# hzxie/Stereo-3D-Reconstruction

Hardware: AMD Instinct MI355X
Metric: stereo pairs/s forward (batch 32, 224x224 -> 32^3 voxel) (higher is better)
Workload: dtype f32

## Files before the change

### stereo-3d-reconstruction_amd/csrc/s3r_conv_wino.hip

```cpp
#include "s3r_kernels.h"
#include <cstdlib>

namespace s3r {

typedef float wf32x16 __attribute__((ext_vector_type(16)));
typedef float wv2f __attribute__((ext_vector_type(2)));
template <int N> struct WVec;
template <> struct WVec<1> { typedef float type; };
template <> struct WVec<2> { typedef wv2f type; };
typedef float wv4f __attribute__((ext_vector_type(4)));
template <> struct WVec<4> { typedef wv4f type; };
template <int N>
__device__ __forceinline__ float wvget(const typename WVec<N>::type& v, int i) {
    if constexpr (N == 1) return v; else return v[i];
}

#define S3R_LDS_PTR_W(p) ((__attribute__((address_space(3))) void*)(p))

#ifndef S3R_WNB
#define S3R_WNB 2
#endif
#ifndef S3R_WBK
#define S3R_WBK 32
#endif
// ... 610 lines not shown
template <int VEC, int KIND, bool HEAD = false, bool XM = false>
__global__ __launch_bounds__(256, (KIND == 1 ? 4 : 3)) void wino_dual_kernel(const ConvParams p) {
    extern __shared__ __attribute__((aligned(16))) float wsmem[];
    if ((int)blockIdx.x < p.big_wgs)
        wino_body<VEC, KIND, 2, false, HEAD, XM>(p, blockIdx.x, p.big_wgs, p.n_begin, p.n_cut, wsmem);
    else
        wino_body<VEC, KIND, 2, true, false, XM>(p, (int)blockIdx.x - p.big_wgs, (int)gridDim.x - p.big_wgs, p.n_cut, p.n_end, wsmem);
}

template <int KIND, bool HEAD>
__global__ __launch_bounds__(256) void wino_finish_kernel(const ConvParams p, const int n_begin, const int n_end, const int npad) {
    constexpr bool DECONV = KIND == 2;
    constexpr int NCLS = WinoKind<KIND>::NCLS, R = WinoKind<KIND>::R;
    const int S = p.Nd * p.Nh * p.Nw;
    const int nn = n_end - n_begin;
    const int pc = DECONV ? (int)blockIdx.y : 0;
    const int rd = (pc >> 2) & 1, rh = (pc >> 1) & 1, rw = pc & 1;
    const float lo = p.act == ACT_RELU ? 0.f : -__builtin_inff();
    constexpr int NBLK = DECONV ? 8 * NCLS : NCLS;
    const int ntl = npad >> 6;
    const float* __restrict__ base = p.part + (size_t)pc * NCLS * 64;
    auto blk = [&](int mm, int nl) { return base + ((size_t)mm * ntl + (nl >> 6)) * (NBLK * 64) + (nl & 63); };
    const long long total = HEAD ? nn : (long long)p.Cout * nn;
    for (long long i = (long long)blockIdx.x * 256 + threadIdx.x; i < total; i += (long long)gridDim.x * 256) {
        const int mrow = HEAD ? 0 : (int)(i / nn);
        const int nl = (int)(i - (long long)mrow * nn);
        const int n = n_begin + nl;
        const int b = p.dS.div(n);
        int rem = n - b * S;
        const int pd = p.dHW.div(rem);
        rem -= pd * p.Nh * p.Nw;
        const int q = p.dW.div(rem);
        const int pw = rem - q * p.Nw;
        int e0, row1 = R;
        if constexpr (DECONV)
            e0 = b * p.y_bs + p.y_org + (2 * pd * p.y_ds + 2 * q * p.y_hs + pw) * 2 + rd * p.y_ds + rh * p.y_hs + rw;
        else {
            e0 = b * p.y_bs + p.y_org + pd * p.y_ds + R * q * p.y_hs + pw;
            row1 = p.Hout - R * q;
        }
        if constexpr (HEAD) {
            float tw[2][R];
#pragma unroll
            for (int wm = 0; wm < 2; ++wm) {
                float th[2][R];
#pragma unroll
                for (int hh = 0; hh < 2; ++hh) {
#pragma unroll
                    for (int k = 0; k < R; ++k) th[hh][k] = 0.f;
                    for (int r = 0; r < 16; ++r) {
                        const int mm = 32 * wm + 4 * hh + (r & 3) + 8 * (r >> 2);
                        if (mm >= p.Cout) continue;
                        const float sc = p.scale ? p.scale[mm] : 1.f, sf = p.shift ? p.shift[mm] : 0.f, hw = p.head_w[mm];
                        float m[NCLS], y[R];
#pragma unroll
                        for (int c = 0; c < NCLS; ++c) m[c] = blk(mm, nl)[c * 64];
                        wino_out<KIND>(m, y);
#pragma unroll
                        for (int k = 0; k < R; ++k) th[hh][k] = fmaf(wino_act(y[k], sc, sf, lo), hw, th[hh][k]);
                    }
                }
#pragma unroll
                for (int k = 0; k < R; ++k) tw[wm][k] = th[0][k] + th[1][k];
            }
            const float hsc = p.head_scale ? p.head_scale[0] : 1.f, hsf = p.head_shift ? p.head_shift[0] : 0.f;
#pragma unroll
            for (int k = 0; k < R; ++k)
                p.y[e0 + wino_out_off<KIND>(k, p.y_ds, p.y_hs)] = wino_head_act(fmaf(tw[0][k] + tw[1][k], hsc, hsf), p.head_act);
        } else {
            const float sc = p.scale ? p.scale[mrow] : 1.f, sf = p.shift ? p.shift[mrow] : 0.f;
            float m[NCLS], y[R];
#pragma unroll
            for (int c = 0; c < NCLS; ++c) m[c] = blk(mrow, nl)[c * 64];
            wino_out<KIND>(m, y);
            float* __restrict__ yo = p.y + (size_t)mrow * p.y_cs + e0;
#pragma unroll
            for (int k = 0; k < R; ++k)
                if (k < row1) yo[wino_out_off<KIND>(k, p.y_ds, p.y_hs)] = wino_act(y[k], sc, sf, lo);
        }
    }
}

template <int KIND>
static hipError_t launch_wino_finish(const ConvParams& p, int n_begin, int n_end, int npad, hipStream_t stream) {
    const long long total = p.head_w ? (long long)(n_end - n_begin) : (long long)p.Cout * (n_end - n_begin);
    const long long blocks = (total + 255) / 256;
    const dim3 grid((unsigned)(blocks < 8192 ? blocks : 8192), KIND == 2 ? 8 : 1);
    if constexpr (KIND == 2) {
        if (p.head_w) hipLaunchKernelGGL((wino_finish_kernel<KIND, true>), grid, dim3(256), 0, stream, p, n_begin, n_end, npad);
        else hipLaunchKernelGGL((wino_finish_kernel<KIND, false>), grid, dim3(256), 0, stream, p, n_begin, n_end, npad);
    } else {
        hipLaunchKernelGGL((wino_finish_kernel<KIND, false>), grid, dim3(256), 0, stream, p, n_begin, n_end, npad);
    }
    return hipGetLastError();
}

constexpr int WCN = 64;
#ifdef S3R_ABLATE
static int wabl_mode() { static const int m = getenv("S3R_ABL") ? atoi(getenv("S3R_ABL")) : 0; return m; }
#define S3R_WABL(p) (p).debug = wabl_mode()
#else
#define S3R_WABL(p) (void)0
#endif

int64_t wino_slab_elems(int kind, int cout, int ntotal, const WinoLaunch& L) {
    if (L.mode == WINO_SERIAL) return 0;
    const int ncls = kind == 2 ? 72 : 6;
    const int n0 = L.mode == WINO_DUAL ? L.n_cut : 0;
    const int64_t npad = (int64_t)((ntotal - n0 + WCN - 1) / WCN) * WCN;
    return (int64_t)ncls * cout * npad;
}

WinoLaunch wino_plan(int kind, int cout, int kcls, int ntotal, bool head, int forced) {
    WinoLaunch L;
    L.mode = WINO_SERIAL; L.n_cut = 0;
    const int m_tiles = (cout + WBM - 1) / WBM;
    const int pcs = kind == 2 ? 8 : 1;
    const int ncls = kind == 2 ? 9 : 6;
    const long W = (long)m_tiles * ((ntotal + WCN - 1) / WCN) * pcs;
    if (forced < 0) {
        static const int env_mode = getenv("S3R_WINO_FORM") ? atoi(getenv("S3R_WINO_FORM")) : -1;
        forced = env_mode;
    }
    const int occ = kind == 2 ? 3 : 4;
    const int CUS = cu_count();
    const double u = (double)W / (double)CUS;
    int kb = (int)u;
    if (forced >= 0) {
        L.mode = forced <= WINO_DUAL ? forced : WINO_SERIAL;
        if ((double)kb >= u) kb -= 1;
    } else {
        (void)head;
        constexpr double EFF = 0.9, EFF_ALONE = 0.7, SLAB = 100.0, LAUNCH = 220.0, TAIL = 0.6;
        const double unit = (double)ncls * kcls;
        auto serial_cost = [&](int w) {
            const int rem = w % occ;
            return (w - (rem == 1 ? 1 : 0)) * unit / EFF + (rem == 1 ? unit / EFF_ALONE : 0.0);
        };
        const double serial = serial_cost((int)__builtin_ceil(u));
        const double cp = __builtin_ceil(u * ncls) * (kcls / EFF + SLAB) + LAUNCH;
        double best = serial;
        if (cp < best) { best = cp; L.mode = WINO_CP; }
        for (int k : {(int)u, (int)u % occ == 1 ? (int)u - 1 : 0}) {
            if (k < 1 || (double)k >= u) continue;
            const double dual = serial_cost(k) + TAIL * __builtin_ceil((u - k) * ncls) * (kcls / EFF + SLAB) + LAUNCH;
            if (dual < 0.97 * best) { best = dual; L.mode = WINO_DUAL; kb = k; }
        }
    }
    if (L.mode == WINO_DUAL) {
        const long n_main = ((long)kb * CUS) / (m_tiles * pcs);
        L.n_cut = (int)(n_main * WCN);
        if (L.n_cut <= 0 || L.n_cut >= ntotal) { L.mode = L.n_cut <= 0 ? WINO_CP : WINO_SERIAL; L.n_cut = 0; }
    }
    return L;
}

template <int VEC, int KIND>
static hipError_t launch_wino_forms(ConvParams p, const WinoLaunch& L, hipStream_t stream) {
    const int ntotal = p.Ntotal;
    if (p.out_mode && (KIND != 2 || L.mode != WINO_CP)) return hipErrorInvalidValue;
    auto lds_of = [](int bn) { return (size_t)WNB * WBK * (WBM + (KIND == 2 ? 2 : 1) * bn) * sizeof(float); };
    const int pcs = KIND == 2 ? 8 : 1;
    constexpr int NCLS = WinoKind<KIND>::NCLS;
    p.n_begin = 0; p.n_end = ntotal;
    if (L.mode == WINO_SERIAL) {
        const dim3 grid(p.m_tiles * ((ntotal + WCN - 1) / WCN) * pcs);
        if constexpr (KIND == 2) {
            if (p.head_w) {
                if (p.xd_mode) hipLaunchKernelGGL((wino_kernel<VEC, KIND, 2, false, true, true>), grid, dim3(256), lds_of(WCN), stream, p);
                else hipLaunchKernelGGL((wino_kernel<VEC, KIND, 2, false, true, false>), grid, dim3(256), lds_of(WCN), stream, p);
            } else {
                if (p.xd_mode) hipLaunchKernelGGL((wino_kernel<VEC, KIND, 2, false, false, true>), grid, dim3(256), lds_of(WCN), stream, p);
                else hipLaunchKernelGGL((wino_kernel<VEC, KIND, 2, false, false, false>), grid, dim3(256), lds_of(WCN), stream, p);
            }
            return hipGetLastError();
        }
        hipLaunchKernelGGL((wino_kernel<VEC, KIND, 2, false, false>), grid, dim3(256), lds_of(WCN), stream, p);
        return hipGetLastError();
    }
    if (!p.part) return hipErrorInvalidValue;
    const int n0 = L.mode == WINO_DUAL ? L.n_cut : 0;
    const int cp_tiles = (ntotal - n0 + WCN - 1) / WCN;
    const int cp_wgs = p.m_tiles * cp_tiles * NCLS * pcs;
    if (L.mode == WINO_DUAL) {
        p.n_cut = n0;
        p.big_wgs = p.m_tiles * (n0 / WCN) * pcs;
        const dim3 grid(p.big_wgs + cp_wgs);
        if constexpr (KIND == 2) {
            if (p.head_w) {
                if (p.xd_mode) hipLaunchKernelGGL((wino_dual_kernel<VEC, KIND, true, true>), grid, dim3(256), lds_of(WCN), stream, p);
                else hipLaunchKernelGGL((wino_dual_kernel<VEC, KIND, true, false>), grid, dim3(256), lds_of(WCN), stream, p);
            } else {
                if (p.xd_mode) hipLaunchKernelGGL((wino_dual_kernel<VEC, KIND, false, true>), grid, dim3(256), lds_of(WCN), stream, p);
                else hipLaunchKernelGGL((wino_dual_kernel<VEC, KIND, false, false>), grid, dim3(256), lds_of(WCN), stream, p);
            }
        } else {
            hipLaunchKernelGGL((wino_dual_kernel<VEC, KIND>), grid, dim3(256), lds_of(WCN), stream, p);
        }
    } else if (KIND == 2 && p.xd_mode) {
        hipLaunchKernelGGL((wino_kernel<VEC, KIND, 2, true, false, KIND == 2>), dim3(cp_wgs), dim3(256), lds_of(WCN), stream, p);
    } else {
        hipLaunchKernelGGL((wino_kernel<VEC, KIND, 2, true, false>), dim3(cp_wgs), dim3(256), lds_of(WCN), stream, p);
    }
    hipError_t e = hipGetLastError();
    if (e != hipSuccess) return e;
    if (p.out_mode) return launch_wino_handoff(p, 2, p.out_mode - 1, cp_tiles * WCN, stream);
    AuxScope aux(stream, 4.0 * (double)(ntotal - n0) * p.Cout * (pcs * NCLS + (p.head_w ? 0.0 : pcs * WinoKind<KIND>::R)));
    return launch_wino_finish<KIND>(p, n0, ntotal, cp_tiles * WCN, stream);
}

hipError_t launch_conv_wino(ConvParams p, const WinoLaunch& L, hipStream_t stream, int* launches) {
    if (p.Cin % WBK != 0 || p.stride != 1 || p.transposed || p.ksplit != 1 || p.head_w || p.act == ACT_SIGMOID)
        return hipErrorInvalidValue;
    p.kh = 1;
    S3R_WABL(p);
    p.m_tiles = (p.Cout + WBM - 1) / WBM;
    if (launches) *launches = L.mode == WINO_SERIAL ? 1 : 2;
    return p.Nw % 4 == 0 ? launch_wino_forms<4, 1>(p, L, stream) : launch_wino_forms<1, 1>(p, L, stream);
}

hipError_t launch_deconv_wino(ConvParams p, const WinoLaunch& L, hipStream_t stream, int* launches) {
    if (p.Cin % WBK != 0 || !p.transposed || p.ksplit != 1 || !p.xd || p.act == ACT_SIGMOID || (p.head_w && p.Cout > WBM))
        return hipErrorInvalidValue;
    S3R_WABL(p);
    p.m_tiles = (p.Cout + WBM - 1) / WBM;
    if (launches) *launches = L.mode == WINO_SERIAL ? 1 : 2;
    if (p.Nw % 4 != 0) return hipErrorInvalidValue;
    return launch_wino_forms<4, 2>(p, L, stream);
}

template <int AX> struct WAxis;
template <> struct WAxis<0> { static constexpr int N = 6, M = 4, R = 3; };
template <> struct WAxis<1> { static constexpr int N = 5, M = 2, R = 4; };
int wino2_classes(int ax) { return ax == 1 ? 25 : 36; }
int wino2_outputs(int ax) { return ax == 1 ? 2 : 4; }

template <int AX>
__device__ __forceinline__ void wax_bt(const float (&r)[WAxis<AX>::N], float (&v)[WAxis<AX>::N]) {
    if constexpr (AX == 0) wino_rows_to_classes<4>(r, v);
    else {
        v[0] = fmaf(2.f, r[0] - r[2], r[3] - r[1]);
        v[1] = fmaf(-2.f, r[1], r[3] - r[2]);
        v[2] = fmaf(2.f, r[1], fmaf(-3.f, r[2], r[3]));
        v[3] = r[3] - r[1];
        v[4] = fmaf(2.f, r[1] - r[3], r[4] - r[2]);
    }
}
template <int AX>
__device__ __forceinline__ void wax_at(const float (&m)[WAxis<AX>::N], float (&y)[WAxis<AX>::M]) {
    if constexpr (AX == 0) wino_out<1>(m, y);
    else {
        y[0] = ((m[0] + m[1]) + m[2]) + m[3];
        y[1] = fmaf(2.f, m[3], m[1] - m[2]) + m[4];
    }
}
template <int AX>
__device__ __forceinline__ float wax_g(int c, const float (&g)[WAxis<AX>::R]) {
    if constexpr (AX == 0) {
        const float s02 = g[0] + g[2], a = g[0] * (1.f / 24.f) + g[2] * (1.f / 6.f), b12 = g[1] * (1.f / 12.f);
        return c == 0 ? g[0] * 0.25f : c == 1 ? (s02 + g[1]) * (-1.f / 6.f) : c == 2 ? (s02 - g[1]) * (-1.f / 6.f)
             : c == 3 ? a + b12 : c == 4 ? a - b12 : g[2];
    } else {
        const float e = g[0] + g[2], o = g[1] + g[3];
        return c == 0 ? g[0] * 0.5f : c == 1 ? (e + o) * -0.5f : c == 2 ? (o - e) * (1.f / 6.f)
             : c == 3 ? fmaf(g[3], 4.f / 3.f, fmaf(g[2], 2.f / 3.f, fmaf(g[1], 1.f / 3.f, g[0] * (1.f / 6.f)))) : g[3];
    }
}

template <int AX>
__global__ __launch_bounds__(256) void wino2_input_kernel(const float* __restrict__ x, float* __restrict__ V, unsigned total,
                                                          int Dp, int Hp, int Wp, int SD, int SH, FastDiv dW, FastDiv dSH, FastDiv dSD) {
    constexpr int N = WAxis<AX>::N, M = WAxis<AX>::M;
    for (unsigned i = blockIdx.x * 256u + threadIdx.x; i < total; i += gridDim.x * 256u) {
        const unsigned row = (unsigned)dW.div((int)i);
        const int w = (int)(i - row * (unsigned)Wp);
        const unsigned pg = (unsigned)dSH.div((int)row);
        const int sh = (int)(row - pg * (unsigned)SH);
        const unsigned pl = (unsigned)dSD.div((int)pg);
        const int sd = (int)(pg - pl * (unsigned)SD);
        const float* __restrict__ src = x + ((size_t)pl * Dp + M * sd) * Hp * Wp + (size_t)M * sh * Wp + w;
        float t[N][N];
#pragma unroll
        for (int a = 0; a < N; ++a) {
            float r[N], v[N];
#pragma unroll
            for (int b = 0; b < N; ++b)
                r[b] = (M * sd + a < Dp && M * sh + b < Hp) ? src[((size_t)a * Hp + b) * Wp] : 0.f;
            wax_bt<AX>(r, v);
#pragma unroll
            for (int b = 0; b < N; ++b) t[a][b] = v[b];
        }
#pragma unroll
        for (int b = 0; b < N; ++b) {
            float r[N], v[N];
#pragma unroll
            for (int a = 0; a < N; ++a) r[a] = t[a][b];
            wax_bt<AX>(r, v);
#pragma unroll
            for (int a = 0; a < N; ++a) V[(size_t)(a * N + b) * total + i] = v[a];
        }
    }
}

hipError_t launch_wino2_input(const float* x, float* V, int ax, long long planes, int Dp, int Hp, int Wp, int SD, int SH, hipStream_t s) {
    const long long total = planes * SD * SH * Wp;
    if (total >= (1ll << 31) || (ax != 0 && ax != 1)) return hipErrorInvalidValue;
    const long long blocks = (total + 255) / 256;
    const dim3 grid((unsigned)(blocks < 16384 ? blocks : 16384));
    const FastDiv dW((unsigned)Wp), dSH((unsigned)SH), dSD((unsigned)SD);
    if (ax == 0) hipLaunchKernelGGL(wino2_input_kernel<0>, grid, dim3(256), 0, s, x, V, (unsigned)total, Dp, Hp, Wp, SD, SH, dW, dSH, dSD);
    else hipLaunchKernelGGL(wino2_input_kernel<1>, grid, dim3(256), 0, s, x, V, (unsigned)total, Dp, Hp, Wp, SD, SH, dW, dSH, dSD);
    return hipGetLastError();
}

template <int AX>
__global__ void pack_wino2_kernel(const float* __restrict__ w, float* __restrict__ wp, int Cin, int Cout, int CoutPad) {
    constexpr int N = WAxis<AX>::N, R = WAxis<AX>::R;
    const size_t per_cls = (size_t)R * Cin * CoutPad;
    for (size_t i = blockIdx.x * (size_t)blockDim.x + threadIdx.x; i < (size_t)N * N * per_cls; i += (size_t)gridDim.x * blockDim.x) {
        const int cls = (int)(i / per_cls);
        const int ca = cls / N, cb = cls - ca * N;
        size_t r = i % per_cls;
        const int co = (int)(r % CoutPad);
        r /= CoutPad;
        const int c = (int)(r % WBK);
        r /= WBK;
        const int tw = (int)(r % R);
        const int cc = (int)(r / R);
        const int cin = cc * WBK + c;
        float v = 0.f;
        if (co < Cout) {
            const float* g = w + ((size_t)co * Cin + cin) * R * R * R + tw;
            float gd[R];
#pragma unroll
            for (int kd = 0; kd < R; ++kd) {
                float gh[R];
#pragma unroll
                for (int kh = 0; kh < R; ++kh) gh[kh] = g[(kd * R + kh) * R];
                gd[kd] = wax_g<AX>(cb, gh);
            }
            v = wax_g<AX>(ca, gd);
        }
        wp[i] = v;
    }
}

__global__ void pack_wino2p_kernel(const float* __restrict__ w, float* __restrict__ wp, int Cin, int Cout, int CoutPad);
hipError_t launch_pack_wino2(const float* w, float* wp, int ax, int Cin, int Cout, int CoutPad, hipStream_t s) {
    if (ax == 0) hipLaunchKernelGGL(pack_wino2_kernel<0>, dim3(1024), dim3(256), 0, s, w, wp, Cin, Cout, CoutPad);
    else if (ax == 1) hipLaunchKernelGGL(pack_wino2_kernel<1>, dim3(1024), dim3(256), 0, s, w, wp, Cin, Cout, CoutPad);
    else if (ax == 2) hipLaunchKernelGGL(pack_wino2p_kernel, dim3(1024), dim3(256), 0, s, w, wp, Cin, Cout, CoutPad);
    else return hipErrorInvalidValue;
    return hipGetLastError();
}

__device__ __forceinline__ void wino2_copy_out(const float* __restrict__ lds, float* __restrict__ dst, int count, int tid) {
    if ((count & 3) == 0 && (reinterpret_cast<size_t>(dst) & 15) == 0) {
        for (int i = tid * 4; i < count; i += 1024) *reinterpret_cast<wv4f*>(dst + i) = *reinterpret_cast<const wv4f*>(lds + i);
    } else {
        for (int i = tid; i < count; i += 256) dst[i] = lds[i];
    }
}
__device__ __forceinline__ void wino2_zero_out(float* __restrict__ dst, int count, int tid) {
    if ((count & 3) == 0 && (reinterpret_cast<size_t>(dst) & 15) == 0) {
        for (int i = tid * 4; i < count; i += 1024) *reinterpret_cast<wv4f*>(dst + i) = wv4f{0.f, 0.f, 0.f, 0.f};
    } else {
        for (int i = tid; i < count; i += 256) dst[i] = 0.f;
    }
}

__global__ __launch_bounds__(256) void wino2s_finish_kernel(const ConvParams p, const int npad, const int halo, const int SUB,
                                                            const FastDiv dNd, const FastDiv dMS) {
    constexpr int N = 6, M = 4;
    extern __shared__ __attribute__((aligned(16))) float fsm[];
    const int tid = threadIdx.x;
    const int G = p.Nh * p.Nw, Wp = p.y_hs, slice = p.y_ds, MS = M * slice;
    const float lo = p.act == ACT_RELU ? 0.f : -__builtin_inff();
    const int per_c = p.B * p.Nd;
    const int nrg = (per_c + SUB - 1) / SUB;
    const bool vec = (slice & 3) == 0 && (reinterpret_cast<size_t>(p.y) & 15) == 0;
    for (int item = blockIdx.x; item < p.Cout * nrg; item += gridDim.x) {
        const int mrow = item / nrg;
        const int r0 = (item - mrow * nrg) * SUB;
        const int nsub = per_c - r0 < SUB ? per_c - r0 : SUB;
        for (int i = tid; i < nsub * MS; i += 256) fsm[i] = 0.f;
        __syncthreads();
        const float sc = p.scale ? p.scale[mrow] : 1.f, sf = p.shift ? p.shift[mrow] : 0.f;
        for (int t = tid; t < nsub * G; t += 256) {
            const int sub = p.dHW.div(t);
            const int g = t - sub * G;
            const int sh = p.dW.div(g);
            const int pw = g - sh * p.Nw;
            const int r = r0 + sub;
            const int sd = r - dNd.div(r) * p.Nd;
            const int n = r0 * G + t;
            const float* __restrict__ src = p.part + ((size_t)mrow * (npad >> 6) + (n >> 6)) * (N * M * 64) + (n & 63);
            float* __restrict__ o = fsm + sub * MS + (halo + M * sh) * Wp + halo + pw;
#pragma unroll
            for (int v = 0; v < M; ++v) {
                float m[N], y[M];
#pragma unroll
                for (int a = 0; a < N; ++a) m[a] = src[(a * M + v) * 64];
                wax_at<0>(m, y);
#pragma unroll
                for (int u = 0; u < M; ++u)
                    if (M * sd + u < p.Dout && M * sh + v < p.Hout) o[u * slice + v * Wp] = wino_act(y[u], sc, sf, lo);
            }
        }
        __syncthreads();
        float* __restrict__ yc = p.y + (size_t)mrow * p.y_cs;
        for (int e = vec ? tid * 4 : tid; e < nsub * MS; e += vec ? 1024 : 256) {
            const int sub = dMS.div(e);
            const int off = e - sub * MS;
            const int r = r0 + sub;
            const int b = dNd.div(r);
            const int sd = r - b * p.Nd;
            const int nsl = p.Dout - M * sd < M ? p.Dout - M * sd : M;
            if (off >= nsl * slice) continue;
            float* __restrict__ dst = yc + (size_t)b * p.y_bs + (size_t)(halo + M * sd) * slice + off;
            if (vec) *reinterpret_cast<wv4f*>(dst) = *reinterpret_cast<const wv4f*>(fsm + e);
            else *dst = fsm[e];
        }
        if (halo > 0)
            for (int sub = 0; sub < nsub; ++sub) {
                const int r = r0 + sub;
                const int b = dNd.div(r);
                const int sd = r - b * p.Nd;
                if (sd == 0) wino2_zero_out(yc + (size_t)b * p.y_bs, halo * slice, tid);
                if (sd == p.Nd - 1) wino2_zero_out(yc + (size_t)b * p.y_bs + (size_t)(halo + p.Dout) * slice, halo * slice, tid);
            }
        __syncthreads();
    }
}

template <int AX>
__global__ __launch_bounds__(256) void wino2_finish_flat_kernel(const ConvParams p, const int npad) {
    constexpr int N = WAxis<AX>::N, M = WAxis<AX>::M;
    const int S = p.Nd * p.Nh * p.Nw;
    const int nn = p.Ntotal;
    const float lo = p.act == ACT_RELU ? 0.f : -__builtin_inff();
    const long long total = (long long)p.Cout * nn;
    for (long long i = (long long)blockIdx.x * 256 + threadIdx.x; i < total; i += (long long)gridDim.x * 256) {
        const int mrow = (int)(i / nn);
        const int n = (int)(i - (long long)mrow * nn);
        const int b = p.dS.div(n);
        int rem = n - b * S;
        const int sd = p.dHW.div(rem);
        rem -= sd * p.Nh * p.Nw;
        const int sh = p.dW.div(rem);
        const int pw = rem - sh * p.Nw;
        const float* __restrict__ src = p.part + ((size_t)mrow * (npad >> 6) + (n >> 6)) * (N * N * 64) + (n & 63);
        float t[N][M];
#pragma unroll
        for (int a = 0; a < N; ++a) {
            float m[N], y[M];
#pragma unroll
            for (int c = 0; c < N; ++c) m[c] = src[(a * N + c) * 64];
            wax_at<AX>(m, y);
#pragma unroll
            for (int v = 0; v < M; ++v) t[a][v] = y[v];
        }
        const float sc = p.scale ? p.scale[mrow] : 1.f, sf = p.shift ? p.shift[mrow] : 0.f;
        float* __restrict__ yo = p.y + (size_t)b * p.y_bs + (size_t)mrow * p.y_cs + p.y_org + (size_t)M * sd * p.y_ds + M * sh * p.y_hs + pw;
#pragma unroll
        for (int v = 0; v < M; ++v) {
            float m[N], y[M];
#pragma unroll
            for (int a = 0; a < N; ++a) m[a] = t[a][v];
            wax_at<AX>(m, y);
#pragma unroll
            for (int u = 0; u < M; ++u)
                if (M * sd + u < p.Dout && M * sh + v < p.Hout) yo[(size_t)u * p.y_ds + v * p.y_hs] = wino_act(y[u], sc, sf, lo);
        }
    }
}

__global__ __launch_bounds__(256) void wino2p_input_kernel(const float* __restrict__ x, float* __restrict__ V, unsigned total, int Cin,
                                                           int Hp, int Wp, int SH, int SW, unsigned npad, unsigned nn, FastDiv dSW,
                                                           FastDiv dSH, FastDiv dN) {
    constexpr int N = 6, M = 4;
    const size_t cstride = (size_t)Cin * npad;
    for (unsigned i = blockIdx.x * 256u + threadIdx.x; i < total; i += gridDim.x * 256u) {
        const unsigned c = (unsigned)dN.div((int)i);
        const unsigned n = i - c * nn;
        const unsigned row = (unsigned)dSW.div((int)n);
        const int sw = (int)(n - row * (unsigned)SW);
        const unsigned b = (unsigned)dSH.div((int)row);
        const int sh = (int)(row - b * (unsigned)SH);
        const float* __restrict__ src = x + (((size_t)b * Cin + c) * Hp + M * sh) * Wp + M * sw;
        float t[N][N];
#pragma unroll
        for (int jc = 0; jc < N; ++jc) {
            float r[N], v[N];
#pragma unroll
            for (int ir = 0; ir < N; ++ir) r[ir] = (M * sh + ir < Hp && M * sw + jc < Wp) ? src[(size_t)ir * Wp + jc] : 0.f;
            wax_bt<0>(r, v);
#pragma unroll
            for (int ir = 0; ir < N; ++ir) t[ir][jc] = v[ir];
        }
        float* __restrict__ dst = V + (size_t)c * npad + n;
#pragma unroll
        for (int bb = 0; bb < N; ++bb) {
            float v[N];
            wax_bt<0>(t[bb], v);
#pragma unroll
            for (int a = 0; a < N; ++a) dst[(size_t)(a * N + bb) * cstride] = v[a];
        }
    }
}

typedef float wv4f_u __attribute__((ext_vector_type(4), aligned(4)));
__global__ __launch_bounds__(256) void wino2p_input_lds_kernel(const float* __restrict__ x, float* __restrict__ V, int B, int Cin, int Hp,
                                                               int Wp, int SH, int SW, int NS, unsigned npad) {
    extern __shared__ __attribute__((aligned(16))) float w2p_sx[];
    constexpr int N = 6, M = 4;
    const int c = blockIdx.x % Cin, b0 = (blockIdx.x / Cin) * NS;
    const int ns = B - b0 < NS ? B - b0 : NS;
    const int plane = Hp * Wp, G = SH * SW;
    for (int sidx = 0; sidx < ns; ++sidx) {
        const float* __restrict__ src = x + ((size_t)(b0 + sidx) * Cin + c) * plane;
        float* dstp = w2p_sx + sidx * plane;
        if ((plane & 3) == 0) {
            for (int i = threadIdx.x; i < plane / 4; i += 256)
                reinterpret_cast<wv4f*>(dstp)[i] = reinterpret_cast<const wv4f_u*>(src)[i];
        } else {
            for (int i = threadIdx.x; i < plane; i += 256) dstp[i] = src[i];
        }
    }
    __syncthreads();
    const int t = threadIdx.x;
    if (t >= ns * G) return;
    const int sidx = t / G, g = t - sidx * G;
    const int sh = g / SW, sw = g - sh * SW;
    const float* __restrict__ src = w2p_sx + sidx * plane + (M * sh) * Wp + M * sw;
    const size_t cstride = (size_t)Cin * npad;
    float tt[N][N];
#pragma unroll
    for (int jc = 0; jc < N; ++jc) {
        float r[N], v[N];
#pragma unroll
        for (int ir = 0; ir < N; ++ir) r[ir] = (M * sh + ir < Hp && M * sw + jc < Wp) ? src[ir * Wp + jc] : 0.f;
        wax_bt<0>(r, v);
#pragma unroll
        for (int ir = 0; ir < N; ++ir) tt[ir][jc] = v[ir];
    }
    float* __restrict__ dst = V + (size_t)c * npad + (size_t)(b0 + sidx) * G + g;
#pragma unroll
    for (int bb = 0; bb < N; ++bb) {
        float v[N];
        wax_bt<0>(tt[bb], v);
#pragma unroll
        for (int a2 = 0; a2 < N; ++a2) dst[(size_t)(a2 * N + bb) * cstride] = v[a2];
    }
}

hipError_t launch_wino2p_input(const float* x, float* V, int B, int Cin, int Hp, int Wp, int SH, int SW, long long npad, hipStream_t s) {
    const long long nn = (long long)B * SH * SW, total = nn * Cin;
    if (total >= (1ll << 31) || npad >= (1ll << 31)) return hipErrorInvalidValue;
    const int G = SH * SW;
    if (G <= 256) {
        int NS = 256 / G;
        if (NS > B) NS = B;
        while (NS > 1 && (size_t)NS * Hp * Wp * 4 > 48 * 1024) --NS;
        const size_t lds = (size_t)NS * Hp * Wp * 4;
        if (lds <= 48 * 1024) {
            const long long blocks = (long long)Cin * ((B + NS - 1) / NS);
            if (blocks < (1ll << 31)) {
                hipLaunchKernelGGL(wino2p_input_lds_kernel, dim3((unsigned)blocks), dim3(256), lds, s, x, V, B, Cin, Hp, Wp, SH, SW, NS,
                                   (unsigned)npad);
                return hipGetLastError();
            }
        }
    }
    const long long blocks = (total + 255) / 256;
    const dim3 grid((unsigned)(blocks < 16384 ? blocks : 16384));
    hipLaunchKernelGGL(wino2p_input_kernel, grid, dim3(256), 0, s, x, V, (unsigned)total, Cin, Hp, Wp, SH, SW, (unsigned)npad, (unsigned)nn,
                       FastDiv((unsigned)SW), FastDiv((unsigned)SH), FastDiv((unsigned)nn));
    return hipGetLastError();
}

__global__ void pack_wino2p_kernel(const float* __restrict__ w, float* __restrict__ wp, int Cin, int Cout, int CoutPad) {
    const size_t per_cls = (size_t)Cin * CoutPad;
    for (size_t i = blockIdx.x * (size_t)blockDim.x + threadIdx.x; i < 36 * per_cls; i += (size_t)gridDim.x * blockDim.x) {
        const int cls = (int)(i / per_cls);
        const int ca = cls / 6, cb = cls - ca * 6;
        const size_t r = i % per_cls;
        const int co = (int)(r % CoutPad);
        const int cin = (int)(r / CoutPad);
        float v = 0.f;
        if (co < Cout) {
            const float* g = w + ((size_t)co * Cin + cin) * 9;
            float gh[3];
#pragma unroll
            for (int kh = 0; kh < 3; ++kh) {
                const float gw[3] = {g[kh * 3], g[kh * 3 + 1], g[kh * 3 + 2]};
                gh[kh] = wax_g<0>(ca, gw);
            }
            v = wax_g<0>(cb, gh);
        }
        wp[i] = v;
    }
}

template <bool SEMI, bool TOV>
__global__ __launch_bounds__(256) void wino2p_finish_kernel(const ConvParams p, const int npad, const int halo, const int PL) {
    constexpr int N = 6, M = 4;
    extern __shared__ __attribute__((aligned(16))) float fsm[];
    const int tid = threadIdx.x;
    const int G = p.Nh * p.Nw, Wp = TOV ? p.Hout + 2 : p.y_hs, plane = TOV ? Wp * Wp : p.y_cs;
    const float lo = p.act == ACT_RELU ? 0.f : -__builtin_inff();
    const size_t cstride = (size_t)p.Cout * npad;
    const int nbg = (p.B + PL - 1) / PL;
    for (int item = blockIdx.x; item < p.Cout * nbg; item += gridDim.x) {
        const int mrow = item / nbg;
        const int b0 = (item - mrow * nbg) * PL;
        const int npl = p.B - b0 < PL ? p.B - b0 : PL;
        for (int i = tid; i < npl * plane; i += 256) fsm[i] = 0.f;
        __syncthreads();
        const float sc = p.scale ? p.scale[mrow] : 1.f, sf = p.shift ? p.shift[mrow] : 0.f;
        for (int t = tid; t < npl * G; t += 256) {
            const int pl = p.dS.div(t);
            const int s = t - pl * G;
            const int sh = p.dW.div(s);
            const int sw = s - sh * p.Nw;
            const int n = b0 * G + t;
            const float* __restrict__ src = p.part + ((size_t)mrow * (npad >> 6) + (n >> 6)) * ((SEMI ? N * M : N * N) * 64) + (n & 63);
            float tt[N][M];
#pragma unroll
            for (int a = 0; a < N; ++a) {
                if constexpr (SEMI) {
#pragma unroll
                    for (int v = 0; v < M; ++v) tt[a][v] = src[(a * M + v) * 64];
                } else {
                    float m[N], y[M];
#pragma unroll
                    for (int c = 0; c < N; ++c) m[c] = src[(a * N + c) * 64];
                    wax_at<0>(m, y);
#pragma unroll
                    for (int v = 0; v < M; ++v) tt[a][v] = y[v];
                }
            }
            float* __restrict__ o = fsm + pl * plane + (halo + M * sh) * Wp + halo + M * sw;
#pragma unroll
            for (int v = 0; v < M; ++v) {
                float m[N], y[M];
#pragma unroll
                for (int a = 0; a < N; ++a) m[a] = tt[a][v];
                wax_at<0>(m, y);
#pragma unroll
                for (int u = 0; u < M; ++u)
                    if (M * sh + v < p.Hout && M * sw + u < p.Hout) o[v * Wp + u] = wino_act(y[u], sc, sf, lo);
            }
        }
        __syncthreads();
        if constexpr (TOV) {
            for (int t = tid; t < npl * G; t += 256) {
                const int pl = p.dS.div(t);
                const int s = t - pl * G;
                const int sh = p.dW.div(s);
                const int sw = s - sh * p.Nw;
                const float* __restrict__ win = fsm + pl * plane + M * sh * Wp + M * sw;
                float tt[N][N];
#pragma unroll
                for (int jc = 0; jc < N; ++jc) {
                    float r[N], v[N];
#pragma unroll
                    for (int ir = 0; ir < N; ++ir) r[ir] = win[ir * Wp + jc];
                    wax_bt<0>(r, v);
#pragma unroll
                    for (int ir = 0; ir < N; ++ir) tt[ir][jc] = v[ir];
                }
                float* __restrict__ dst = p.y + (size_t)mrow * npad + (size_t)b0 * G + t;
#pragma unroll
                for (int bb = 0; bb < N; ++bb) {
                    float v[N];
                    wax_bt<0>(tt[bb], v);
#pragma unroll
                    for (int a = 0; a < N; ++a) dst[(size_t)(a * N + bb) * cstride] = v[a];
                }
            }
        } else {
            for (int pl = 0; pl < npl; ++pl)
                wino2_copy_out(fsm + pl * plane, p.y + (size_t)(b0 + pl) * p.y_bs + (size_t)mrow * p.y_cs, plane, tid);
        }
        __syncthreads();
    }
}

template <int PROD, int CONS>
__global__ __launch_bounds__(256) void wino_handoff_kernel(const ConvParams p, const int npad, const int CB, const int On, const int halo,
                                                           const int SG, const FastDiv dG1, const FastDiv dG2, const FastDiv dOp,
                                                           const FastDiv dOp2, const FastDiv dSG) {
    extern __shared__ __attribute__((aligned(16))) float hsm[];
    const int tid = threadIdx.x;
    const int Op = On + 2 * halo, hs = Op, ds = Op * Op, vol = ds * Op, org = halo * (ds + hs + 1);
    const int S = p.Nd * p.Nh * p.Nw;
    const int G1 = PROD == 2 ? 8 * S : S;
    const int G2 = CONS == 2 ? vol : SG * SG * Op;
    const int ncb = (p.Cout + CB - 1) / CB;
    const float lo = p.act == ACT_RELU ? 0.f : -__builtin_inff();
    const bool vec2 = CONS == 2 && (Op & 1) == 0 && (reinterpret_cast<size_t>(p.y) & 7) == 0;
    for (int item = blockIdx.x; item < p.B * ncb; item += gridDim.x) {
        const int b = item / ncb;
        const int c0 = (item - b * ncb) * CB;
        const int nc = p.Cout - c0 < CB ? p.Cout - c0 : CB;
        for (int i = tid; i < nc * vol; i += 256) hsm[i] = 0.f;
        __syncthreads();
        for (int t = tid; t < nc * G1; t += 256) {
            const int cl = dG1.div(t);
            int g = t - cl * G1;
            const int mrow = c0 + cl;
            const float sc = p.scale ? p.scale[mrow] : 1.f, sf = p.shift ? p.shift[mrow] : 0.f;
            float* __restrict__ o = hsm + cl * vol + org;
            if constexpr (PROD <= 1) {
                constexpr int N = WAxis<PROD>::N, M = WAxis<PROD>::M;
                const int n = b * S + g;
                const int sd = p.dHW.div(g);
                g -= sd * p.Nh * p.Nw;
                const int sh = p.dW.div(g);
                const int pw = g - sh * p.Nw;
                const float* __restrict__ src = p.part + ((size_t)mrow * (npad >> 6) + (n >> 6)) * (N * N * 64) + (n & 63);
                float tt[N][M];
#pragma unroll
                for (int a = 0; a < N; ++a) {
                    float m[N], y[M];
#pragma unroll
                    for (int c = 0; c < N; ++c) m[c] = src[(a * N + c) * 64];
                    wax_at<PROD>(m, y);
#pragma unroll
                    for (int v = 0; v < M; ++v) tt[a][v] = y[v];
                }
                o += M * sd * ds + M * sh * hs + pw;
#pragma unroll
                for (int v = 0; v < M; ++v) {
                    float m[N], y[M];
#pragma unroll
                    for (int a = 0; a < N; ++a) m[a] = tt[a][v];
                    wax_at<PROD>(m, y);
#pragma unroll
                    for (int u = 0; u < M; ++u)
                        if (M * sd + u < p.Dout && M * sh + v < p.Hout) o[u * ds + v * hs] = wino_act(y[u], sc, sf, lo);
                }
            } else if constexpr (PROD == 2) {
                constexpr int NCLS = WinoKind<2>::NCLS, R = WinoKind<2>::R;
                const int pc = p.dS.div(g);
                g -= pc * S;
                const int rd = (pc >> 2) & 1, rh = (pc >> 1) & 1, rw = pc & 1;
                const int n = b * S + g;
                const int pd = p.dHW.div(g);
                g -= pd * p.Nh * p.Nw;
                const int q = p.dW.div(g);
                const int pw = g - q * p.Nw;
                const float* __restrict__ src = p.part + (size_t)pc * NCLS * 64 + ((size_t)mrow * (npad >> 6) + (n >> 6)) * (8 * NCLS * 64) + (n & 63);
                float m[NCLS], y[R];
#pragma unroll
                for (int c = 0; c < NCLS; ++c) m[c] = src[c * 64];
                wino_out<2>(m, y);
                o += (2 * pd * ds + 2 * q * hs + pw) * 2 + rd * ds + rh * hs + rw;
#pragma unroll
                for (int k = 0; k < R; ++k) o[wino_out_off<2>(k, ds, hs)] = wino_act(y[k], sc, sf, lo);
            } else {
                const int n = b * S + g;
                const float* __restrict__ src = p.part + (size_t)mrow * npad + n;
                const size_t zs = (size_t)p.Cout * npad;
                float sum = src[0];
                for (int z = 1; z < p.ksplit; ++z) sum += src[(size_t)z * zs];
                const int pd = p.dHW.div(g);
                g -= pd * p.Nh * p.Nw;
                const int ph = p.dW.div(g);
                const int pw = g - ph * p.Nw;
                float t1 = fmaf(sum, sc, sf);
                if (p.act == ACT_RELU) t1 = fmaxf(t1, fmaf(t1, p.slope, 0.f));
                o[pd * ds + ph * hs + pw] = t1;
            }
        }
        __syncthreads();
        const size_t base = ((size_t)b * p.Cout + c0) * G2;
        const size_t total = (size_t)p.B * p.Cout * G2;
        for (int t = tid; t < (CONS == 2 && vec2 ? 0 : nc * G2); t += 256) {
            const int cl = dG2.div(t);
            const int e = t - cl * G2;
            if constexpr (CONS <= 1) {
                constexpr int N = WAxis<CONS>::N, M = WAxis<CONS>::M;
                const int row = dOp.div(e);
                const int w = e - row * Op;
                const int sd = dSG.div(row);
                const int sh = row - sd * SG;
                const float* __restrict__ src = hsm + cl * vol + M * sd * ds + M * sh * hs + w;
                float tt[N][N];
#pragma unroll
                for (int a = 0; a < N; ++a) {
                    float r[N], v[N];
#pragma unroll
                    for (int c = 0; c < N; ++c) r[c] = (M * sd + a < Op && M * sh + c < Op) ? src[a * ds + c * hs] : 0.f;
                    wax_bt<CONS>(r, v);
#pragma unroll
                    for (int c = 0; c < N; ++c) tt[a][c] = v[c];
                }
#pragma unroll
                for (int c = 0; c < N; ++c) {
                    float r[N], v[N];
#pragma unroll
                    for (int a = 0; a < N; ++a) r[a] = tt[a][c];
                    wax_bt<CONS>(r, v);
#pragma unroll
                    for (int a = 0; a < N; ++a) p.y[(size_t)(a * N + c) * total + base + t] = v[a];
                }
            } else if (!vec2) {
                const int z = dOp2.div(e);
                const int r = dOp.div(e - z * ds);
                const bool rn = r + 1 < Op, zn = z + 1 < Op;
                const float* __restrict__ src = hsm + t;
                const float x00 = src[0];
                const float x01 = rn ? src[hs] : 0.f;
                const float dh0 = rn ? x00 - x01 : 0.f;
                const float x10 = zn ? src[ds] : 0.f;
                const float x11 = (rn && zn) ? src[ds + hs] : 0.f;
                const float dh1 = rn ? x10 - x11 : 0.f;
                float* __restrict__ dst = p.y + base + t;
                dst[0] = x00;
                dst[total] = dh0;
                dst[2 * total] = zn ? x00 - x10 : 0.f;
                dst[3 * total] = zn ? dh0 - dh1 : 0.f;
            }
        }
        if constexpr (CONS == 2) {
            if (vec2)
                for (int t = tid * 2; t < nc * G2; t += 512) {
                    const int cl = dG2.div(t);
                    const int e = t - cl * G2;
                    const int z = dOp2.div(e);
                    const int r = dOp.div(e - z * ds);
                    const bool rn = r + 1 < Op, zn = z + 1 < Op;
                    const wv2f zero = {0.f, 0.f};
                    const float* __restrict__ src = hsm + t;
                    const wv2f x00 = *reinterpret_cast<const wv2f*>(src);
                    const wv2f x01 = rn ? *reinterpret_cast<const wv2f*>(src + hs) : zero;
                    const wv2f dh0 = rn ? x00 - x01 : zero;
                    const wv2f x10 = zn ? *reinterpret_cast<const wv2f*>(src + ds) : zero;
                    const wv2f x11 = (rn && zn) ? *reinterpret_cast<const wv2f*>(src + ds + hs) : zero;
                    const wv2f dh1 = rn ? x10 - x11 : zero;
                    float* __restrict__ dst = p.y + base + t;
                    *reinterpret_cast<wv2f*>(dst) = x00;
                    *reinterpret_cast<wv2f*>(dst + total) = dh0;
                    *reinterpret_cast<wv2f*>(dst + 2 * total) = zn ? x00 - x10 : zero;
                    *reinterpret_cast<wv2f*>(dst + 3 * total) = zn ? dh0 - dh1 : zero;
                }
        }
        __syncthreads();
    }
}

hipError_t launch_wino_handoff(const ConvParams& p, int prod, int cons, int npad, hipStream_t stream) {
    if (prod < 0 || prod > 3 || cons < 0 || cons > 2 || !p.part || !p.y || npad <= 0 || (npad & 63) || p.head_w) return hipErrorInvalidValue;
    const int Op = p.y_hs;
    if (Op <= 0 || p.y_ds != Op * Op || p.y_cs != Op * Op * Op || p.y_bs != p.Cout * p.y_cs) return hipErrorInvalidValue;
    const int halo = p.y_org / (p.y_ds + p.y_hs + 1), On = Op - 2 * halo;
    if (p.y_org != halo * (p.y_ds + p.y_hs + 1) || On <= 0) return hipErrorInvalidValue;
    if ((cons == 0 && (halo != 1 || On < 4)) || (cons == 1 && (halo != 0 || On < 5)) || (cons == 2 && (halo != 1 || (On & 3)))) return hipErrorInvalidValue;
    const int SG = cons == 0 ? (On + 3) / 4 : cons == 1 ? (On - 2) / 2 : 1;
    const int vol = Op * Op * Op;
    if (vol > 8192) return hipErrorInvalidValue;
    const int CB = 8192 / vol < 8 ? 8192 / vol : 8;
    const int S = p.Nd * p.Nh * p.Nw;
    if (p.Ntotal != p.B * S || npad < p.Ntotal) return hipErrorInvalidValue;
    double slabs;
    if (prod <= 1) {
        if (p.ncls != wino2_classes(prod) || p.Dout != On || p.Hout != On || p.Nw != On || p.act == ACT_SIGMOID) return hipErrorInvalidValue;
        slabs = (double)p.ncls * npad;
    } else if (prod == 2) {
        if (!p.transposed || cons != 2 || 2 * p.Nw != On || 4 * p.Nd != On || 4 * p.Nh != On || p.act == ACT_SIGMOID) return hipErrorInvalidValue;
        slabs = 72.0 * npad;
    } else {
        if (p.transposed || cons == 2 || p.ksplit <= 1 || p.y_step > 1 || p.shuf_s || p.Nd != On || p.Nh != On || p.Nw != On || p.act == ACT_SIGMOID)
            return hipErrorInvalidValue;
        slabs = (double)p.ksplit * npad;
    }
    const int G1 = prod == 2 ? 8 * S : S, G2 = cons == 2 ? vol : SG * SG * Op;
    const double written = cons == 2 ? 4.0 * p.B * vol : (double)wino2_classes(cons) * p.B * G2;
    if ((double)p.Cout * written >= 2147483648.0) return hipErrorInvalidValue;
    const long long items = (long long)p.B * ((p.Cout + CB - 1) / CB);
    const dim3 grid((unsigned)(items < 16384 ? items : 16384));
    const size_t lds = (size_t)CB * vol * sizeof(float);
    const FastDiv dG1((unsigned)G1), dG2((unsigned)G2), dOp((unsigned)Op), dOp2((unsigned)(Op * Op)), dSG((unsigned)SG);
    AuxScope aux(stream, 4.0 * (double)p.Cout * (slabs + written));
#define S3R_HANDOFF(PR, CO) hipLaunchKernelGGL((wino_handoff_kernel<PR, CO>), grid, dim3(256), lds, stream, p, npad, CB, On, halo, SG, dG1, dG2, dOp, dOp2, dSG)
    switch (prod * 3 + cons) {
        case 0: S3R_HANDOFF(0, 0); break;
        case 1: S3R_HANDOFF(0, 1); break;
        case 2: S3R_HANDOFF(0, 2); break;
        case 3: S3R_HANDOFF(1, 0); break;
        case 4: S3R_HANDOFF(1, 1); break;
        case 5: S3R_HANDOFF(1, 2); break;
        case 8: S3R_HANDOFF(2, 2); break;
        case 9: S3R_HANDOFF(3, 0); break;
        case 10: S3R_HANDOFF(3, 1); break;
        default: return hipErrorInvalidValue;
    }
#undef S3R_HANDOFF
    return hipGetLastError();
}

int wino2_form(int ax, int cout, int ntotal, int forced) {
    if (ax == 1) return 0;
    if (forced >= 0) return forced ? 1 : 0;
    static const int env_form = getenv("S3R_WINO2_FORM") ? atoi(getenv("S3R_WINO2_FORM")) : -1;
    if (env_form >= 0) return env_form ? 1 : 0;
    const long semi_wgs = (long)((cout + WBM - 1) / WBM) * ((ntotal + WCN - 1) / WCN) * 6;
    return semi_wgs >= (ax == 2 ? 2 : 8) * (long)cu_count() ? 1 : 0;
}
int64_t wino2_npad(int64_t ntotal) { return (ntotal + WCN - 1) / WCN * WCN; }
int64_t wino2_slab_elems(int ax, int cout, int ntotal, int form) {
    const int64_t npad = (int64_t)((ntotal + WCN - 1) / WCN) * WCN;
    return (form ? 6 * 4 : wino2_classes(ax)) * (int64_t)cout * npad;
}

hipError_t launch_conv_wino2(ConvParams p, int ax, int form, bool to_v, hipStream_t stream, int* launches) {
    if (p.Cin % WBK != 0 || p.stride != 1 || p.transposed || p.ksplit != 1 || p.head_w || p.act == ACT_SIGMOID || !p.part ||
        ax < 0 || ax > 2 || p.ncls != wino2_classes(ax))
        return hipErrorInvalidValue;
    p.kh = 1;
    S3R_WABL(p);
    p.m_tiles = (p.Cout + WBM - 1) / WBM;
    p.n_begin = 0; p.n_end = p.Ntotal;
    const int n_tiles = (p.Ntotal + WCN - 1) / WCN;
    const size_t lds = (size_t)WNB * WBK * (WBM + WCN) * sizeof(float);
    const int halo = to_v ? 1 : (p.y_hs - p.Hout) / 2;
    if (to_v && (ax != 2 || p.Hout % 4 != 0)) return hipErrorInvalidValue;
    if (p.out_mode && (to_v || ax == 2 || form != 0)) return hipErrorInvalidValue;
    if (!to_v && (halo < 0 || p.y_hs != p.Hout + 2 * halo)) return hipErrorInvalidValue;
    if (ax == 2) {
        const int plane = to_v ? (p.Hout + 2) * (p.Hout + 2) : p.y_hs * p.y_hs, G = p.Nh * p.Nw;
        if ((!to_v && p.y_cs != plane) || (size_t)plane * 4 > 64 * 1024) return hipErrorInvalidValue;
        int PL = 256 / G < 1 ? 1 : 256 / G;
        if (PL > p.B) PL = p.B;
        while (PL > 1 && (size_t)PL * plane * 4 > 64 * 1024) --PL;
        const int npad = n_tiles * WCN;
        ConvParams q = p;
        q.B = 1; q.Nd = 1; q.Nh = 1; q.Nw = npad;
        q.dS = q.dHW = q.dW = FastDiv((unsigned)npad);
        q.kd = q.kh = q.kw = 1; q.T = 1;
        q.x_org = 0; q.x_ds = 0; q.x_hs = 0; q.x_cs = npad; q.x_cls = p.Cin * npad;
        q.x_bytes = (unsigned)(4ull * 36 * p.Cin * npad);
        q.Ntotal = npad; q.n_end = npad;
        const dim3 grid(p.m_tiles * n_tiles * (form == 1 ? 6 : 36));
        if (form == 1) hipLaunchKernelGGL((wino_kernel<4, 1, 2, false, false, false, true>), grid, dim3(256), lds, stream, q);
        else hipLaunchKernelGGL((wino_kernel<4, 1, 2, true, false>), grid, dim3(256), lds, stream, q);
        hipError_t e = hipGetLastError();
        if (e != hipSuccess) return e;
        const long long items = (long long)p.Cout * ((p.B + PL - 1) / PL);
        const dim3 fgrid((unsigned)(items < 16384 ? items : 16384));
        const size_t flds = (size_t)PL * plane * 4;
        AuxScope aux(stream, 4.0 * (double)p.Cout * ((double)(form == 1 ? 24 : 36) * npad + (to_v ? 36.0 * npad : (double)p.B * plane)));
        if (to_v) {
            if (form == 1) hipLaunchKernelGGL((wino2p_finish_kernel<true, true>), fgrid, dim3(256), flds, stream, p, npad, halo, PL);
            else hipLaunchKernelGGL((wino2p_finish_kernel<false, true>), fgrid, dim3(256), flds, stream, p, npad, halo, PL);
        } else if (form == 1) hipLaunchKernelGGL((wino2p_finish_kernel<true, false>), fgrid, dim3(256), flds, stream, p, npad, halo, PL);
        else hipLaunchKernelGGL((wino2p_finish_kernel<false, false>), fgrid, dim3(256), flds, stream, p, npad, halo, PL);
        if (launches) *launches = 2;
        return hipGetLastError();
    }
    if (p.y_ds != p.y_hs * p.y_hs || p.y_cs != (p.Dout + 2 * halo) * p.y_ds) return hipErrorInvalidValue;
    if (form == 1) {
        const int M = wino2_outputs(ax), G = p.Nh * p.Nw;
        if (ax != 0 || (size_t)M * p.y_ds * 4 > 64 * 1024) return hipErrorInvalidValue;
        int SUB = 256 / G < 1 ? 1 : 256 / G;
        if (SUB > p.B * p.Nd) SUB = p.B * p.Nd;
        while (SUB > 1 && (size_t)SUB * M * p.y_ds * 4 > 64 * 1024) --SUB;
        const size_t flds = (size_t)SUB * M * p.y_ds * 4;
        const FastDiv dNd((unsigned)p.Nd), dMS((unsigned)(M * p.y_ds));
        const long long items = (long long)p.Cout * ((p.B * p.Nd + SUB - 1) / SUB);
        const dim3 fgrid((unsigned)(items < 32768 ? items : 32768));
        const dim3 grid(p.m_tiles * n_tiles * 6);
        if (p.Nw % 4 == 0) hipLaunchKernelGGL((wino_kernel<4, 1, 2, false, false, false, true>), grid, dim3(256), lds, stream, p);
        else hipLaunchKernelGGL((wino_kernel<1, 1, 2, false, false, false, true>), grid, dim3(256), lds, stream, p);
        hipError_t e = hipGetLastError();
        if (e != hipSuccess) return e;
        AuxScope aux(stream, 4.0 * (double)p.Cout * (24.0 * n_tiles * WCN + (double)p.B * p.y_cs));
        hipLaunchKernelGGL(wino2s_finish_kernel, fgrid, dim3(256), flds, stream, p, n_tiles * WCN, halo, SUB, dNd, dMS);
        if (launches) *launches = 2;
        return hipGetLastError();
    }
    const dim3 grid(p.m_tiles * n_tiles * p.ncls);
    if (p.Nw % 4 == 0) hipLaunchKernelGGL((wino_kernel<4, 1, 2, true, false>), grid, dim3(256), lds, stream, p);
    else hipLaunchKernelGGL((wino_kernel<1, 1, 2, true, false>), grid, dim3(256), lds, stream, p);
    hipError_t e = hipGetLastError();
    if (e != hipSuccess) return e;
    if (launches) *launches = 2;
    if (p.out_mode) return launch_wino_handoff(p, ax, p.out_mode - 1, n_tiles * WCN, stream);
    const long long total = (long long)p.Cout * p.Ntotal;
    const long long blocks = (total + 255) / 256;
    const dim3 flat((unsigned)(blocks < 8192 ? blocks : 8192));
    AuxScope aux(stream, 4.0 * (double)p.Cout * ((double)p.ncls * n_tiles * WCN + (double)p.B * p.Dout * p.Hout * p.Nw));
    if (ax == 0) hipLaunchKernelGGL(wino2_finish_flat_kernel<0>, flat, dim3(256), 0, stream, p, n_tiles * WCN);
    else hipLaunchKernelGGL(wino2_finish_flat_kernel<1>, flat, dim3(256), 0, stream, p, n_tiles * WCN);
    if (launches) *launches = 2;
    return hipGetLastError();
}

#ifdef S3R_ABLATE
}
extern "C" int s3r_debug_read_timeline_wino(unsigned long long* out, int nblocks) {
    if (nblocks > 65536) nblocks = 65536;
    return hipMemcpyFromSymbol(out, HIP_SYMBOL(s3r::s3r_wino_timeline), sizeof(unsigned long long) * 6 * (size_t)nblocks) == hipSuccess ? nblocks : -1;
}
extern "C" int s3r_debug_clear_timeline_wino() {
    void* ptr = nullptr;
    if (hipGetSymbolAddress(&ptr, HIP_SYMBOL(s3r::s3r_wino_timeline)) != hipSuccess) return -1;
    return hipMemset(ptr, 0, sizeof(unsigned long long) * 6 * 65536) == hipSuccess ? 0 : -1;
}
namespace s3r {
#endif

}
```

Before: 8818.

## Stage Winograd input planes in LDS and vectorize semi-Winograd finish kernel

Result: no change. 8859 (median of 6 runs) (+0.5%).

```diff
diff --git a/stereo-3d-reconstruction_amd/csrc/s3r_conv_wino.hip b/stereo-3d-reconstruction_amd/csrc/s3r_conv_wino.hip
--- a/stereo-3d-reconstruction_amd/csrc/s3r_conv_wino.hip
+++ b/stereo-3d-reconstruction_amd/csrc/s3r_conv_wino.hip
@@ -936,9 +936,106 @@
     }
 }
 
+static int wino2_env() {
+    static const int v = getenv("S3R_WINO2_FORM") ? atoi(getenv("S3R_WINO2_FORM")) : -1;
+    return v;
+}
+
+typedef float wv4f_u __attribute__((ext_vector_type(4), aligned(4)));
+template <int AX>
+__global__ __launch_bounds__(256) void wino2_input_lds_kernel(const float* __restrict__ x, float* __restrict__ V, unsigned total,
+                                                              int planes, int Dp, int Hp, int Wp, int SD, int SH, int NV, int LW,
+                                                              FastDiv dW, FastDiv dSH, FastDiv dSD) {
+    constexpr int N = WAxis<AX>::N, M = WAxis<AX>::M;
+    extern __shared__ __attribute__((aligned(16))) float w2i_sx[];
+    const int pl0 = blockIdx.x * NV;
+    const int nv = planes - pl0 < NV ? planes - pl0 : NV;
+    const int rows = Dp * Hp, vol = rows * Wp, volL = rows * LW;
+    const float* __restrict__ xs = x + (size_t)pl0 * vol;
+    if ((Wp & 3) == 0) {
+        constexpr int U = 8;
+        for (int i0 = threadIdx.x * 4; i0 < nv * vol; i0 += 1024 * U) {
+            wv4f pv[U];
+#pragma unroll
+            for (int u = 0; u < U; ++u) {
+                const int i = i0 + u * 1024;
+                pv[u] = *reinterpret_cast<const wv4f_u*>(xs + (i < nv * vol ? i : 0));
+            }
+#pragma unroll
+            for (int u = 0; u < U; ++u) {
+                const int i = i0 + u * 1024;
+                const int row = dW.div(i);
+                if (i < nv * vol) *reinterpret_cast<wv4f*>(w2i_sx + row * LW + (i - row * Wp)) = pv[u];
+            }
+        }
+    } else {
+        for (int i = threadIdx.x; i < nv * vol; i += 256) {
+            const int row = dW.div(i);
+            w2i_sx[row * LW + (i - row * Wp)] = xs[i];
+        }
+    }
+    __syncthreads();
+    const int per = SD * SH * Wp;
+    for (int t = threadIdx.x; t < nv * per; t += 256) {
+        const unsigned i = (unsigned)pl0 * (unsigned)per + (unsigned)t;
+        const int row = dW.div(t);
+        const int w = t - row * Wp;
+        const int pg = dSH.div(row);
+        const int sh = row - pg * SH;
+        const int v = dSD.div(pg);
+        const int sd = pg - v * SD;
+        const float* __restrict__ src = w2i_sx + v * volL + ((M * sd) * Hp + M * sh) * LW + w;
+        float tt[N][N];
+#pragma unroll
+        for (int a = 0; a < N; ++a) {
+            float r[N], c[N];
+#pragma unroll
+            for (int b = 0; b < N; ++b)
+                r[b] = (M * sd + a < Dp && M * sh + b < Hp) ? src[(a * Hp + b) * LW] : 0.f;
+            wax_bt<AX>(r, c);
+#pragma unroll
+            for (int b = 0; b < N; ++b) tt[a][b] = c[b];
+        }
+#pragma unroll
+        for (int b = 0; b < N; ++b) {
+            float r[N], c[N];
+#pragma unroll
+            for (int a = 0; a < N; ++a) r[a] = tt[a][b];
+            wax_bt<AX>(r, c);
+#pragma unroll
+            for (int a = 0; a < N; ++a) V[(size_t)(a * N + b) * total + i] = c[a];
+        }
+    }
+}
+
+static int wino2_input_lds_plan(int ax, long long planes, int Dp, int Hp, int Wp, int* LW) {
+    const int M = wino2_outputs(ax);
+    int lw = (Wp + 3) & ~3;
+    if ((M * lw) % 32 != 16) lw += 4;
+    *LW = lw;
+    const long long vol_bytes = 4ll * Dp * Hp * lw;
+    long long nv = (48 * 1024) / vol_bytes;
+    if (nv > planes) nv = planes;
+    return (int)nv;
+}
+
 hipError_t launch_wino2_input(const float* x, float* V, int ax, long long planes, int Dp, int Hp, int Wp, int SD, int SH, hipStream_t s) {
     const long long total = planes * SD * SH * Wp;
     if (total >= (1ll << 31) || (ax != 0 && ax != 1)) return hipErrorInvalidValue;
+    int LW = 0;
+    const int NV = wino2_env() == 2 ? 0 : wino2_input_lds_plan(ax, planes, Dp, Hp, Wp, &LW);
+    if (NV > 0) {
+        const dim3 grid((unsigned)((planes + NV - 1) / NV));
+        const size_t lds = (size_t)NV * Dp * Hp * LW * 4;
+        const FastDiv dW((unsigned)Wp), dSH((unsigned)SH), dSD((unsigned)SD);
+        if (ax == 0)
+            hipLaunchKernelGGL(wino2_input_lds_kernel<0>, grid, dim3(256), lds, s, x, V, (unsigned)total, (int)planes, Dp, Hp, Wp, SD, SH, NV, LW,
+                               dW, dSH, dSD);
+        else
+            hipLaunchKernelGGL(wino2_input_lds_kernel<1>, grid, dim3(256), lds, s, x, V, (unsigned)total, (int)planes, Dp, Hp, Wp, SD, SH, NV, LW,
+                               dW, dSH, dSD);
+        return hipGetLastError();
+    }
     const long long blocks = (total + 255) / 256;
     const dim3 grid((unsigned)(blocks < 16384 ? blocks : 16384));
     const FastDiv dW((unsigned)Wp), dSH((unsigned)SH), dSD((unsigned)SD);
@@ -1003,6 +1100,7 @@
     }
 }
 
+template <int VEC>
 __global__ __launch_bounds__(256) void wino2s_finish_kernel(const ConvParams p, const int npad, const int halo, const int SUB,
                                                             const FastDiv dNd, const FastDiv dMS) {
     constexpr int N = 6, M = 4;
@@ -1017,10 +1115,23 @@
         const int mrow = item / nrg;
         const int r0 = (item - mrow * nrg) * SUB;
         const int nsub = per_c - r0 < SUB ? per_c - r0 : SUB;
-        for (int i = tid; i < nsub * MS; i += 256) fsm[i] = 0.f;
-        __syncthreads();
+        if constexpr (VEC == 4) {
+            const int Hp = slice / Wp;
+            for (int i = tid; i < nsub * M * Hp; i += 256) {
+                float* __restrict__ row = fsm + i * Wp;
+                const int rr = i - (i / Hp) * Hp;
+                if (rr < halo || rr >= Hp - halo) {
+                    for (int c = 0; c < Wp; ++c) row[c] = 0.f;
+                } else {
+                    for (int c = 0; c < halo; ++c) { row[c] = 0.f; row[Wp - 1 - c] = 0.f; }
+                }
+            }
+        } else {
+            for (int i = tid; i < nsub * MS; i += 256) fsm[i] = 0.f;
+            __syncthreads();
+        }
         const float sc = p.scale ? p.scale[mrow] : 1.f, sf = p.shift ? p.shift[mrow] : 0.f;
-        for (int t = tid; t < nsub * G; t += 256) {
+        for (int t = tid * VEC; t < nsub * G; t += 256 * VEC) {
             const int sub = p.dHW.div(t);
             const int g = t - sub * G;
             const int sh = p.dW.div(g);
@@ -1030,15 +1141,35 @@
             const int n = r0 * G + t;
             const float* __restrict__ src = p.part + ((size_t)mrow * (npad >> 6) + (n >> 6)) * (N * M * 64) + (n & 63);
             float* __restrict__ o = fsm + sub * MS + (halo + M * sh) * Wp + halo + pw;
-#pragma unroll
-            for (int v = 0; v < M; ++v) {
-                float m[N], y[M];
-#pragma unroll
-                for (int a = 0; a < N; ++a) m[a] = src[(a * M + v) * 64];
-                wax_at<0>(m, y);
-#pragma unroll
-                for (int u = 0; u < M; ++u)
-                    if (M * sd + u < p.Dout && M * sh + v < p.Hout) o[u * slice + v * Wp] = wino_act(y[u], sc, sf, lo);
+            if constexpr (VEC == 4) {
+                wv4f q[M][N];
+#pragma unroll
+                for (int v = 0; v < M; ++v)
+#pragma unroll
+                    for (int a = 0; a < N; ++a) q[v][a] = *reinterpret_cast<const wv4f_u*>(src + (a * M + v) * 64);
+#pragma unroll
+                for (int v = 0; v < M; ++v)
+#pragma unroll
+                    for (int j = 0; j < 4; ++j) {
+                        float m[N], y[M];
+#pragma unroll
+                        for (int a = 0; a < N; ++a) m[a] = q[v][a][j];
+                        wax_at<0>(m, y);
+#pragma unroll
+                        for (int u = 0; u < M; ++u)
+                            if (M * sd + u < p.Dout && M * sh + v < p.Hout) o[u * slice + v * Wp + j] = wino_act(y[u], sc, sf, lo);
+                    }
+            } else {
+#pragma unroll
+                for (int v = 0; v < M; ++v) {
+                    float m[N], y[M];
+#pragma unroll
+                    for (int a = 0; a < N; ++a) m[a] = src[(a * M + v) * 64];
+                    wax_at<0>(m, y);
+#pragma unroll
+                    for (int u = 0; u < M; ++u)
+                        if (M * sd + u < p.Dout && M * sh + v < p.Hout) o[u * slice + v * Wp] = wino_act(y[u], sc, sf, lo);
+                }
             }
         }
         __syncthreads();
@@ -1143,7 +1274,6 @@
     }
 }
 
-typedef float wv4f_u __attribute__((ext_vector_type(4), aligned(4)));
 __global__ __launch_bounds__(256) void wino2p_input_lds_kernel(const float* __restrict__ x, float* __restrict__ V, int B, int Cin, int Hp,
                                                                int Wp, int SH, int SW, int NS, unsigned npad) {
     extern __shared__ __attribute__((aligned(16))) float w2p_sx[];
@@ -1538,8 +1668,8 @@
 int wino2_form(int ax, int cout, int ntotal, int forced) {
     if (ax == 1) return 0;
     if (forced >= 0) return forced ? 1 : 0;
-    static const int env_form = getenv("S3R_WINO2_FORM") ? atoi(getenv("S3R_WINO2_FORM")) : -1;
-    if (env_form >= 0) return env_form ? 1 : 0;
+    const int env_form = wino2_env();
+    if (env_form == 0 || env_form == 1) return env_form;
     const long semi_wgs = (long)((cout + WBM - 1) / WBM) * ((ntotal + WCN - 1) / WCN) * 6;
     return semi_wgs >= (ax == 2 ? 2 : 8) * (long)cu_count() ? 1 : 0;
 }
@@ -1598,9 +1728,10 @@
     if (form == 1) {
         const int M = wino2_outputs(ax), G = p.Nh * p.Nw;
         if (ax != 0 || (size_t)M * p.y_ds * 4 > 64 * 1024) return hipErrorInvalidValue;
-        int SUB = 256 / G < 1 ? 1 : 256 / G;
+        const int FV = p.Nw % 4 == 0 && wino2_env() != 2 ? 4 : 1;
+        int SUB = 256 * FV / G < 1 ? 1 : 256 * FV / G;
         if (SUB > p.B * p.Nd) SUB = p.B * p.Nd;
-        while (SUB > 1 && (size_t)SUB * M * p.y_ds * 4 > 64 * 1024) --SUB;
+        while (SUB > 1 && (size_t)SUB * M * p.y_ds * 4 > (FV == 4 ? 32 : 64) * 1024) --SUB;
         const size_t flds = (size_t)SUB * M * p.y_ds * 4;
         const FastDiv dNd((unsigned)p.Nd), dMS((unsigned)(M * p.y_ds));
         const long long items = (long long)p.Cout * ((p.B * p.Nd + SUB - 1) / SUB);
@@ -1611,7 +1742,8 @@
         hipError_t e = hipGetLastError();
         if (e != hipSuccess) return e;
         AuxScope aux(stream, 4.0 * (double)p.Cout * (24.0 * n_tiles * WCN + (double)p.B * p.y_cs));
-        hipLaunchKernelGGL(wino2s_finish_kernel, fgrid, dim3(256), flds, stream, p, n_tiles * WCN, halo, SUB, dNd, dMS);
+        if (FV == 4) hipLaunchKernelGGL(wino2s_finish_kernel<4>, fgrid, dim3(256), flds, stream, p, n_tiles * WCN, halo, SUB, dNd, dMS);
+        else hipLaunchKernelGGL(wino2s_finish_kernel<1>, fgrid, dim3(256), flds, stream, p, n_tiles * WCN, halo, SUB, dNd, dMS);
         if (launches) *launches = 2;
         return hipGetLastError();
     }
```
